# irvingzhang0512/tf_eager_object_detection

Measured on AMD Instinct MI355X. Metric: images/sec, higher is better.
Workload: dtype f32

## Files before the change

tf_eager_object_detection_amd/csrc/postops.hip:

```cpp
#include <mutex>

#include "odet_internal.h"

#define PO_THREADS 1024
#define PO_ROUND 128

typedef unsigned long long u64;

static int next_pow2_(int v) {
  int p = 1;
  while (p < v) p <<= 1;
  return p;
}

struct PostOpsParams {
  PerImg<const float*> scores_t;
  PerImg<const float*> deltas_t;
  PerImg<const float4*> rois_t;
  PerImg<const int32_t*> count_dev_t;
  int R, Ccls, P2, K;
  float means[4], stds[4];
  float wmax, hmax, min_edge, score_thr, nms_thr;
  float roi_div;
  PerImg<int32_t*> cls_count_t;
  PerImg<float4*> cls_boxes_t;
  PerImg<float*> cls_scores_t;
  PerImg<uint32_t*> ticket_t;
  int ncls1, max_per_image;
  int mode;
  PerImg<float4*> out_boxes_t;
  PerImg<int32_t*> out_labels_t;
  PerImg<float*> out_scores_t;
  PerImg<int32_t*> out_count_t;
  PerImg<float*> out_record_t;
};

__device__ __forceinline__ float key_to_score(uint32_t k) {
  const uint32_t asc = ~k;
  const uint32_t u = (asc & 0x80000000u) ? (asc & 0x7FFFFFFFu) : ~asc;
  return __uint_as_float(u);
}

struct MergeView {
  const int32_t* cls_count; const float4* cls_boxes; const float* cls_scores;
  int ncls1, K, max_per_image, mode;
  float4* out_boxes; int32_t* out_labels; float* out_scores; int32_t* out_count; float* out_record;
};

__device__ void postops_merge(const MergeView& p, unsigned char* smem) {
  uint32_t* key = reinterpret_cast<uint32_t*>(smem);
  const int nslots = p.ncls1 * p.K;
  uint32_t* hist = key + nslots;
  uint32_t* sel_key = hist + 256;
  uint32_t* sel_slot = sel_key + (p.max_per_image > 0 ? p.max_per_image : 1);
  __shared__ uint32_t s_prefix, s_target, s_total;
  __shared__ int lds17[17];
  const int tid = threadIdx.x, lane = tid & 63;
  const int per = (nslots + PO_THREADS - 1) / PO_THREADS;
  const int lo = tid * per;
  int nvalid = 0;
  for (int q = 0; q < per; ++q) {
    const int slot = lo + q;
    if (slot < nslots) {
      const int c = slot / p.K, k = slot - c * p.K;
      const float sc = p.cls_scores[slot];
      const bool valid = k < min(p.cls_count[c], p.K);
      key[slot] = valid ? ~d_float_asc_key(sc) : 0xFFFFFFFFu;
      nvalid += valid ? 1 : 0;
    }
  }
  int total;
  (void)block_excl_scan(nvalid, lds17, &total);
  const int M = (p.mode == 1) ? ((p.max_per_image > 0 && total > p.max_per_image) ? p.max_per_image : total)
                              : min(total, p.max_per_image);
  uint32_t T = 0xFFFFFFFFu;
  if (M > 0 && M < total) {
    if (tid == 0) { s_prefix = 0u; s_target = (uint32_t)M; }
    for (int pass = 0; pass < 4; ++pass) {
      const int shift = 24 - 8 * pass;
      if (tid < 256) hist[tid] = 0u;
      __syncthreads();
      const uint32_t prefix = s_prefix;
      const uint32_t himask = pass == 0 ? 0u : (0xFFFFFFFFu << (shift + 8));
      for (int q = 0; q < per; ++q) {
        const int slot = lo + q;
        if (slot < nslots) {
          const uint32_t k = key[slot];
          if (k != 0xFFFFFFFFu && (k & himask) == prefix) atomicAdd(&hist[(k >> shift) & 255u], 1u);
        }
      }
      __syncthreads();
      if (tid < 64) {
        const uint32_t h0 = hist[4 * tid], h1 = hist[4 * tid + 1], h2 = hist[4 * tid + 2], h3 = hist[4 * tid + 3];
        const int sum = (int)(h0 + h1 + h2 + h3);
        const int inc = wave_incl_scan(sum);
        const int tgt = (int)s_target;
        const bool hit = sum > 0 && inc - sum < tgt && tgt <= inc;
        const u64 bal = __ballot(hit);
        if (bal && lane == __builtin_ctzll(bal)) {
          int run = inc - sum;
          uint32_t d = 4 * tid;
          const uint32_t hh[4] = {h0, h1, h2, h3};
#pragma unroll
          for (int j = 0; j < 4; ++j) {
            if (run < tgt && tgt <= run + (int)hh[j]) { d = 4 * tid + j; s_target = (uint32_t)(tgt - run); }
            run += (int)hh[j];
          }
          s_prefix = prefix | (d << shift);
        }
      }
      __syncthreads();
    }
    T = s_prefix;
  }
  const uint32_t take_ties = (M > 0 && M < total) ? s_target : 0xFFFFFFFFu;
  __syncthreads();
  if (p.mode == 1) {
    int c = 0;
    for (int q = 0; q < per; ++q) {
      const int slot = lo + q;
      if (slot < nslots && key[slot] != 0xFFFFFFFFu && key[slot] <= T) ++c;
    }
    int kept_total;
    int o = block_excl_scan(c, lds17, &kept_total);
    for (int q = 0; q < per; ++q) {
      const int slot = lo + q;
      if (slot < nslots && key[slot] != 0xFFFFFFFFu && key[slot] <= T) {
        p.out_boxes[o] = p.cls_boxes[slot];
        p.out_scores[o] = p.cls_scores[slot];
        p.out_labels[o] = (int32_t)(slot / p.K) + 1;
        ++o;
      }
    }
    if (tid == 0) *p.out_count = kept_total;
    return;
  }
  int nlt = 0, neq = 0;
  for (int q = 0; q < per; ++q) {
    const int slot = lo + q;
    if (slot < nslots) {
      const uint32_t k = key[slot];
      if (k != 0xFFFFFFFFu) { nlt += (k < T || M == total) ? 1 : 0; neq += (k == T && M < total) ? 1 : 0; }
    }
  }
  int tot_eq, tot_lt;
  int eq_before = block_excl_scan(neq, lds17, &tot_eq);
  int sel_before = block_excl_scan(nlt + max(0, min(neq, (int)min((u64)take_ties, (u64)0x7FFFFFFF) - eq_before)), lds17, &tot_lt);
  {
    int o = sel_before, e = eq_before;
    for (int q = 0; q < per; ++q) {
      const int slot = lo + q;
      if (slot < nslots) {
        const uint32_t k = key[slot];
        bool sel = false;
        if (k != 0xFFFFFFFFu) {
          if (k < T || M == total) sel = true;
          else if (k == T) { sel = (uint32_t)e < take_ties; ++e; }
        }
        if (sel && o < M) { sel_key[o] = k; sel_slot[o] = (uint32_t)slot; ++o; }
      }
    }
  }
  __syncthreads();
  for (int i = tid; i < M; i += PO_THREADS) {
    const uint32_t ki = sel_key[i], si = sel_slot[i];
    int rank = 0;
    for (int j = 0; j < M; ++j) {
      const uint32_t kj = sel_key[j], sj = sel_slot[j];
      rank += (kj < ki || (kj == ki && sj < si)) ? 1 : 0;
    }
    const float4 b = p.cls_boxes[si];
    const float sc = p.cls_scores[si];
    const int lab = (int)(si / (uint32_t)p.K) + 1;
    p.out_boxes[rank] = b;
    p.out_scores[rank] = sc;
    p.out_labels[rank] = lab;
    if (p.out_record) {
      float* r = p.out_record + (size_t)rank * 6;
      r[0] = b.x; r[1] = b.y; r[2] = b.z; r[3] = b.w; r[4] = sc; r[5] = (float)lab;
    }
  }
  if (p.out_record) {
    for (int i = M + tid; i < p.max_per_image; i += PO_THREADS) {
      float* r = p.out_record + (size_t)i * 6;
      r[0] = 0.0f; r[1] = 0.0f; r[2] = 0.0f; r[3] = 0.0f; r[4] = -1.0f; r[5] = 0.0f;
    }
  }
  if (tid == 0) {
    *p.out_count = M;
    if (p.out_record) p.out_record[(size_t)p.max_per_image * 6] = (float)M;
  }
}

__global__ void __launch_bounds__(PO_THREADS) k_postops(PostOpsParams p) {
  extern __shared__ __align__(16) unsigned char smem[];
  const int img = blockIdx.y;
  const float* __restrict__ in_scores = p.scores_t.v[img];
  const float* __restrict__ in_deltas = p.deltas_t.v[img];
  const float4* __restrict__ in_rois = p.rois_t.v[img];
  const int32_t* __restrict__ in_count = p.count_dev_t.v[img];
  int32_t* __restrict__ cls_count = p.cls_count_t.v[img];
  float4* __restrict__ cls_boxes = p.cls_boxes_t.v[img];
  float* __restrict__ cls_scores = p.cls_scores_t.v[img];
  const int nkeys = p.P2 > 2048 ? p.P2 : 2048;
  u64* keys = reinterpret_cast<u64*>(smem);
  float4* lbox = reinterpret_cast<float4*>(keys + nkeys);
  float4* sbox = lbox + p.R;
  float4* kbox = sbox + PO_ROUND;
  u64* mask = reinterpret_cast<u64*>(kbox + p.K);
  float* sarea = reinterpret_cast<float*>(mask + PO_ROUND * 2);
  float* karea = sarea + PO_ROUND;
  uint32_t* crossf = reinterpret_cast<uint32_t*>(karea + p.K);
  __shared__ int s_nvalid, s_nk, s_last;

  const int c = blockIdx.x + 1;
  const int tid = threadIdx.x, lane = tid & 63, w = tid >> 6;
  if (tid == 0) { s_nvalid = 0; s_nk = 0; s_last = 0; }

  const int Rdev = in_count ? *in_count : p.R;
  u64 mykey = ~0ull;
  for (int r = tid; r < p.P2; r += PO_THREADS) {
    u64 key = ~0ull;
    if (r < p.R) {
      const float s = in_scores[(size_t)r * p.Ccls + c];
      const float4 t = *reinterpret_cast<const float4*>(in_deltas + ((size_t)r * p.Ccls + c) * 4);
      float4 roi = in_rois[r];
      if (r < min(Rdev, p.R) && s > p.score_thr) {
        const float d0 = t.x * p.stds[0] + p.means[0];
        const float d1 = t.y * p.stds[1] + p.means[1];
        const float d2 = t.z * p.stds[2] + p.means[2];
        const float d3 = t.w * p.stds[3] + p.means[3];
        if (p.roi_div != 1.0f) {
          roi.x = roi.x / p.roi_div; roi.y = roi.y / p.roi_div; roi.z = roi.z / p.roi_div; roi.w = roi.w / p.roi_div;
        }
        float4 b = d_decode_box(roi, d0, d1, d2, d3);
        b = d_clip_box(b, 0.0f, p.wmax, p.hmax);
        const float e0 = b.z - b.x + 1.0f, e1 = b.w - b.y + 1.0f;
        if (e1 >= p.min_edge && e0 >= p.min_edge) {
          lbox[r] = b;
          key = ((u64)(~d_float_asc_key(s)) << 32) | (unsigned)r;
        }
      }
    }
    if (p.P2 > 1024) keys[r] = key; else mykey = key;
  }
  __syncthreads();
  {
    const u64 bal = __ballot(p.P2 <= 1024 && mykey != ~0ull);
    if (lane == 0 && bal) atomicAdd(&s_nvalid, (int)__popcll(bal));
  }
  __syncthreads();

  if (p.P2 <= 1024) {
    mykey = bitonic_sort_1024_reg(mykey, keys);
    __syncthreads();
    keys[tid] = mykey;
    __syncthreads();
  } else {
    bitonic_sort_u64(keys, p.P2, PO_THREADS);
    if (tid == 0) {
      int lo = 0, hi = p.P2;
      while (lo < hi) { int mid = (lo + hi) >> 1; if (keys[mid] != ~0ull) lo = mid + 1; else hi = mid; }
      s_nvalid = lo;
    }
    __syncthreads();
  }
  const int nvalid = s_nvalid;
  const int K = p.K;

  const u64 lt_lane = (lane == 0) ? 0ull : (~0ull >> (64 - lane));
  for (int t0 = 0; t0 < nvalid; t0 += PO_ROUND) {
    const int nk0 = s_nk;
    if (nk0 >= K) break;
    const int mround = min(PO_ROUND, nvalid - t0);
    if (tid < PO_ROUND) {
      float4 nb = make_float4(0, 0, 0, 0);
      if (tid < mround) nb = d_norm_box(lbox[(int)(keys[t0 + tid] & 0xFFFFFFFFull)]);
      sbox[tid] = nb;
      sarea[tid] = d_box_area(nb);
      crossf[tid] = 0;
    }
    __syncthreads();
    {
      const int row = tid & (PO_ROUND - 1), cs = tid >> 7;
      const float4 rb = sbox[row];
      const float ra = sarea[row];
      uint32_t bits = 0;
#pragma unroll
      for (int j = 0; j < 16; ++j) {
        const int col = cs * 16 + j;
        const bool s = (col < row) && d_iou_gt(rb, ra, sbox[col], sarea[col], p.nms_thr);
        bits |= s ? (1u << j) : 0u;
      }
      reinterpret_cast<unsigned short*>(mask)[row * 8 + cs] = (unsigned short)bits;
      bool sup = false;
      for (int k = cs; k < nk0; k += 8) sup = sup || d_iou_gt(rb, ra, kbox[k], karea[k], p.nms_thr);
      if (sup) atomicOr(&crossf[row], 1u);
    }
    __syncthreads();
    if (w == 0) {
      int nk = nk0;
      u64 kept0 = 0;
#pragma unroll
      for (int blk = 0; blk < 2; ++blk) {
        const int row = blk * 64 + lane;
        const u64 m0 = mask[row * 2 + 0], m1 = mask[row * 2 + 1];
        bool dead = (row >= mround) || (crossf[row] != 0);
        if (blk == 1) dead = dead || ((m0 & kept0) != 0ull);
        const u64 mm = (blk == 0) ? m0 : m1;
        u64 alive = __ballot(!dead);
        u64 kept = 0;
        while (alive != 0 && nk < K) {
          const int i = __builtin_ctzll(alive);
          kept |= 1ull << i;
          ++nk;
          alive &= ~(1ull << i);
          alive &= ~__ballot((mm >> i) & 1ull);
        }
        if (blk == 0) kept0 = kept;
        if ((kept >> lane) & 1ull) {
          const int slot = nk0 + (blk == 1 ? (int)__popcll(kept0) : 0) + (int)__popcll(kept & lt_lane);
          const u64 kk = keys[t0 + row];
          const float4 ob = lbox[(int)(kk & 0xFFFFFFFFull)];
          kbox[slot] = sbox[row];
          karea[slot] = sarea[row];
          cls_boxes[(size_t)blockIdx.x * K + slot] = ob;
          cls_scores[(size_t)blockIdx.x * K + slot] = key_to_score((uint32_t)(kk >> 32));
        }
      }
      if (lane == 0) s_nk = nk;
    }
    __syncthreads();
  }
  if (tid == 0) cls_count[blockIdx.x] = s_nk;

  asm volatile("s_waitcnt vmcnt(0)" ::: "memory");
  __syncthreads();
  if (tid == 0) {
    __builtin_amdgcn_fence(__ATOMIC_RELEASE, "agent");
    asm volatile("s_waitcnt vmcnt(0)" ::: "memory");
    const uint32_t t = atomicInc(p.ticket_t.v[img], (uint32_t)(p.ncls1 - 1));
    s_last = (t == (uint32_t)(p.ncls1 - 1)) ? 1 : 0;
  }
  __syncthreads();
  if (!s_last) return;
  if (tid == 0) __builtin_amdgcn_fence(__ATOMIC_ACQUIRE, "agent");
  asm volatile("s_waitcnt vmcnt(0)" ::: "memory");
  __syncthreads();
  MergeView mv;
  mv.cls_count = cls_count; mv.cls_boxes = cls_boxes; mv.cls_scores = cls_scores;
  mv.ncls1 = p.ncls1; mv.K = p.K; mv.max_per_image = p.max_per_image; mv.mode = p.mode;
  mv.out_boxes = p.out_boxes_t.v[img]; mv.out_labels = p.out_labels_t.v[img]; mv.out_scores = p.out_scores_t.v[img];
  mv.out_count = p.out_count_t.v[img]; mv.out_record = p.out_record_t.v[img];
  postops_merge(mv, smem);
}

extern "C" size_t odet_post_ops_workspace_bytes(int num_classes, int max_per_class) {
  size_t n1 = (size_t)(num_classes > 1 ? num_classes - 1 : 1);
  size_t k = (size_t)(max_per_class > 0 ? max_per_class : 1);
  return odet_align_up(n1 * 4, 256) + odet_align_up(n1 * k * 16, 256) + odet_align_up(n1 * k * 4, 256) + 1024;
}

int odet_post_ops_batch(const PostOpsImageIO* io, int B, int R, int Ccls, int num_classes, PostOpsExtra ex,
                        const float* means, const float* stds, int max_per_class, int max_per_image,
                        float nms_iou_threshold, float score_threshold, float min_edge, hipStream_t st, int ws_clean) {
  ODET_REQUIRE(io && B >= 1 && B <= ODET_MAX_BATCH, "odet_post_ops: bad batch");
  ODET_REQUIRE(R >= 0 && Ccls > 0 && num_classes >= 1 && num_classes <= Ccls, "odet_post_ops: bad sizes");
  ODET_REQUIRE(max_per_class >= 0 && max_per_image >= 0, "odet_post_ops: negative cap");
  for (int i = 0; i < B; ++i) ODET_REQUIRE(io[i].out_count, "odet_post_ops: null out_count");
  if (R == 0 || num_classes == 1 || max_per_class == 0 || (max_per_image == 0 && ex.mode == 0)) {
    for (int i = 0; i < B; ++i) {
      ODET_HIP(hipMemsetAsync(io[i].out_count, 0, sizeof(int32_t), st));
      if (io[i].out_record && max_per_image > 0) {
        int rc = odet_pack_detections(io[i].out_boxes, io[i].out_labels, io[i].out_scores, io[i].out_count, 0,
                                      max_per_image, io[i].out_record, (odet_stream_t)st);
        if (rc != ODET_OK) return rc;
      }
    }
    return ODET_OK;
  }
  ODET_REQUIRE(means && stds, "odet_post_ops: null pointer");
  if (R > ODET_POSTOPS_MAX_ROIS)
    return odet_set_error(ODET_E_LIMIT, "odet_post_ops: R %d exceeds %d", R, ODET_POSTOPS_MAX_ROIS);
  const int ncls1 = num_classes - 1;
  if ((int64_t)ncls1 * max_per_class > ODET_POSTOPS_MAX_CANDIDATES)
    return odet_set_error(ODET_E_LIMIT, "odet_post_ops: (num_classes-1)*max_per_class %lld exceeds %d",
                          (long long)ncls1 * max_per_class, ODET_POSTOPS_MAX_CANDIDATES);
  const size_t need = odet_post_ops_workspace_bytes(num_classes, max_per_class);
  PostOpsParams p;
  for (int i = 0; i < ODET_MAX_BATCH; ++i) {
    const PostOpsImageIO& a = io[i < B ? i : 0];
    ODET_REQUIRE(a.scores && a.deltas && a.rois && a.out_boxes && a.out_labels && a.out_scores,
                 "odet_post_ops: null pointer");
    ODET_REQUIRE((uintptr_t)a.deltas % 16 == 0, "odet_post_ops: deltas must be 16-byte aligned");
    if (!a.workspace || a.workspace_bytes < need)
      return odet_set_error(ODET_E_WORKSPACE, "odet_post_ops: workspace too small (%zu < %zu)", a.workspace_bytes, need);
    OdetArena ar{(char*)a.workspace, a.workspace_bytes, 0};
    int32_t* cc = ar.take<int32_t>(ncls1);
    float4* cb = ar.take<float4>((size_t)ncls1 * max_per_class);
    float* cs = ar.take<float>((size_t)ncls1 * max_per_class);
    uint32_t* tk = ar.take<uint32_t>(1);
    ODET_REQUIRE(cc && cb && cs && tk, "odet_post_ops: workspace arena exhausted");
    p.scores_t.v[i] = a.scores; p.deltas_t.v[i] = a.deltas; p.rois_t.v[i] = (const float4*)a.rois;
    p.count_dev_t.v[i] = a.count_dev;
    p.cls_count_t.v[i] = cc; p.cls_boxes_t.v[i] = cb; p.cls_scores_t.v[i] = cs; p.ticket_t.v[i] = tk;
    p.out_boxes_t.v[i] = (float4*)a.out_boxes; p.out_labels_t.v[i] = a.out_labels; p.out_scores_t.v[i] = a.out_scores;
    p.out_count_t.v[i] = a.out_count; p.out_record_t.v[i] = a.out_record;
    if (!ws_clean && i < B) ODET_HIP(hipMemsetAsync(tk, 0, sizeof(uint32_t), st));
  }
  p.R = R; p.Ccls = Ccls; p.P2 = next_pow2_(R < 2 ? 2 : R); p.K = max_per_class;
  for (int k = 0; k < 4; ++k) { p.means[k] = means[k]; p.stds[k] = stds[k]; }
  p.wmax = ex.wmax; p.hmax = ex.hmax; p.roi_div = ex.roi_div;
  p.min_edge = min_edge; p.score_thr = score_threshold; p.nms_thr = nms_iou_threshold;
  p.ncls1 = ncls1; p.max_per_image = max_per_image; p.mode = ex.mode;
  const size_t nkeys1 = (size_t)(p.P2 > 2048 ? p.P2 : 2048);
  const size_t lds_class = nkeys1 * 8 + (size_t)R * 16 + PO_ROUND * 16 + (size_t)max_per_class * 16 + PO_ROUND * 16 +
                           PO_ROUND * 4 + (size_t)max_per_class * 4 + PO_ROUND * 4;
  const size_t lds_merge = (size_t)ncls1 * max_per_class * 4 + 256 * 4 + (size_t)(max_per_image > 0 ? max_per_image : 1) * 8 + 64;
  const size_t lds1 = lds_class > lds_merge ? lds_class : lds_merge;
  if (lds1 > 150 * 1024)
    return odet_set_error(ODET_E_LIMIT, "odet_post_ops: R/max_per_class need %zu B of LDS (> 150 KiB)", lds1);
  static OdetPerDeviceOnce once;
  ODET_HIP(once.run([] { return hipFuncSetAttribute((const void*)k_postops, hipFuncAttributeMaxDynamicSharedMemorySize, 150 * 1024); }));
  hipLaunchKernelGGL(k_postops, dim3(ncls1, B), dim3(PO_THREADS), lds1, st, p);
  ODET_LAUNCH_CHECK();
  return ODET_OK;
}

static int post_ops_impl(const float* scores, const float* deltas, const float* rois, int R,
                         const int32_t* count_dev, int Ccls, int num_classes, PostOpsExtra ex,
                         const float* means, const float* stds, int max_per_class, int max_per_image,
                         float nms_iou_threshold, float score_threshold, float min_edge, float* out_boxes,
                         int32_t* out_labels, float* out_scores, int32_t* out_count, float* out_record,
                         void* workspace, size_t workspace_bytes, hipStream_t st) {
  PostOpsImageIO io{scores, deltas, rois, count_dev, out_boxes, out_labels, out_scores, out_count, out_record,
                    workspace, workspace_bytes};
  ODET_REQUIRE(out_count, "odet_post_ops: null out_count");
  return odet_post_ops_batch(&io, 1, R, Ccls, num_classes, ex, means, stds, max_per_class, max_per_image,
                             nms_iou_threshold, score_threshold, min_edge, st,  0);
}

extern "C" int odet_post_ops(const float* scores, const float* deltas, const float* rois, int R,
                             const int32_t* count_dev, int Ccls, int num_classes, int image_h, int image_w,
                             const float* means, const float* stds, int max_per_class, int max_per_image,
                             float nms_iou_threshold, float score_threshold, float min_edge, float* out_boxes,
                             int32_t* out_labels, float* out_scores, int32_t* out_count, void* workspace,
                             size_t workspace_bytes, odet_stream_t stream) {
  ODET_REQUIRE(image_h > 0 && image_w > 0, "odet_post_ops: bad image shape");
  return post_ops_impl(scores, deltas, rois, R, count_dev, Ccls, num_classes,
                       PostOpsExtra{(float)(image_w - 1), (float)(image_h - 1), 1.0f, 0}, means, stds,
                       max_per_class, max_per_image, nms_iou_threshold, score_threshold, min_edge, out_boxes,
                       out_labels, out_scores, out_count, nullptr, workspace, workspace_bytes, (hipStream_t)stream);
}

extern "C" int odet_eval_detect(const float* scores, const float* deltas, const float* rois, int R,
                                const int32_t* count_dev, int Ccls, int num_classes, float img_scale, float raw_h,
                                float raw_w, const float* means, const float* stds, int max_per_class,
                                int max_per_image, float nms_iou_threshold, float score_threshold, float min_size,
                                float* out_boxes, int32_t* out_labels, float* out_scores, int32_t* out_count,
                                void* workspace, size_t workspace_bytes, odet_stream_t stream) {
  ODET_REQUIRE(img_scale > 0.0f && raw_h > 0.0f && raw_w > 0.0f, "odet_eval_detect: bad scale / image size");
  return post_ops_impl(scores, deltas, rois, R, count_dev, Ccls, num_classes,
                       PostOpsExtra{raw_w - 1.0f, raw_h - 1.0f, img_scale, 1}, means, stds, max_per_class,
                       max_per_image, nms_iou_threshold, score_threshold, min_size, out_boxes, out_labels,
                       out_scores, out_count, nullptr, workspace, workspace_bytes, (hipStream_t)stream);
}

extern "C" int odet_eval_detect_topk(const float* scores, const float* deltas, const float* rois, int R,
                                     const int32_t* count_dev, int Ccls, int num_classes, float img_scale, float raw_h,
                                     float raw_w, const float* means, const float* stds, int max_per_class,
                                     int max_per_image, float nms_iou_threshold, float score_threshold, float min_size,
                                     float* out_boxes, int32_t* out_labels, float* out_scores, int32_t* out_count,
                                     void* workspace, size_t workspace_bytes, odet_stream_t stream) {
  ODET_REQUIRE(img_scale > 0.0f && raw_h > 0.0f && raw_w > 0.0f, "odet_eval_detect_topk: bad scale / image size");
  return post_ops_impl(scores, deltas, rois, R, count_dev, Ccls, num_classes,
                       PostOpsExtra{raw_w - 1.0f, raw_h - 1.0f, img_scale, 0}, means, stds, max_per_class,
                       max_per_image, nms_iou_threshold, score_threshold, min_size, out_boxes, out_labels,
                       out_scores, out_count, nullptr, workspace, workspace_bytes, (hipStream_t)stream);
}

extern "C" int odet_post_ops_record(const float* scores, const float* deltas, const float* rois, int R,
                                    const int32_t* count_dev, int Ccls, int num_classes, int image_h, int image_w,
                                    const float* means, const float* stds, int max_per_class, int max_per_image,
                                    float nms_iou_threshold, float score_threshold, float min_edge,
                                    float* out_boxes, int32_t* out_labels, float* out_scores, int32_t* out_count,
                                    float* out_record, void* workspace, size_t workspace_bytes,
                                    odet_stream_t stream) {
  ODET_REQUIRE(out_record, "odet_post_ops_record: null out_record");
  ODET_REQUIRE(image_h > 0 && image_w > 0, "odet_post_ops_record: bad image shape");
  return post_ops_impl(scores, deltas, rois, R, count_dev, Ccls, num_classes,
                       PostOpsExtra{(float)(image_w - 1), (float)(image_h - 1), 1.0f, 0}, means, stds,
                       max_per_class, max_per_image, nms_iou_threshold, score_threshold, min_edge, out_boxes,
                       out_labels, out_scores, out_count, out_record, workspace, workspace_bytes,
                       (hipStream_t)stream);
}

__global__ void __launch_bounds__(256) k_pack_detections(const float4* __restrict__ boxes,
                                                         const int32_t* __restrict__ labels,
                                                         const float* __restrict__ scores,
                                                         const int32_t* __restrict__ count, int cap, int max_det,
                                                         float* __restrict__ rec) {
  const int m = min(min(*count, cap), max_det);
  for (int i = threadIdx.x; i < max_det; i += 256) {
    float* r = rec + (size_t)i * 6;
    if (i < m) {
      float4 b = boxes[i];
      r[0] = b.x; r[1] = b.y; r[2] = b.z; r[3] = b.w; r[4] = scores[i]; r[5] = (float)labels[i];
    } else {
      r[0] = 0.0f; r[1] = 0.0f; r[2] = 0.0f; r[3] = 0.0f; r[4] = -1.0f; r[5] = 0.0f;
    }
  }
  if (threadIdx.x == 0) rec[(size_t)max_det * 6] = (float)m;
}

extern "C" int odet_pack_detections(const float* boxes, const int32_t* labels, const float* scores,
                                    const int32_t* count_dev, int capacity, int max_det, float* out_record,
                                    odet_stream_t stream) {
  ODET_REQUIRE(boxes && labels && scores && count_dev && out_record, "odet_pack_detections: null pointer");
  ODET_REQUIRE(capacity >= 0 && max_det > 0, "odet_pack_detections: bad sizes");
  hipLaunchKernelGGL(k_pack_detections, dim3(1), dim3(256), 0, (hipStream_t)stream, (const float4*)boxes, labels,
                     scores, count_dev, capacity, max_det, out_record);
  ODET_LAUNCH_CHECK();
  return ODET_OK;
}
```

Baseline: 29620.

## Replace full bitonic sort with per-round radix select and lazy box decode

The per-class NMS kernel no longer sorts all R candidate keys with a bitonic sort and decodes every box up front. Each round it picks the next top PO_ROUND candidates with a four-pass radix select, ranks them within the round, and decodes only those boxes. Block size and round size drop to 512 threads and 64 rows, which shrinks LDS use and may allow more blocks per CU. The cost is a radix select pass over all R keys every round, which can add up when many rounds run before K boxes are kept.

```diff
diff --git a/tf_eager_object_detection_amd/csrc/postops.hip b/tf_eager_object_detection_amd/csrc/postops.hip
--- a/tf_eager_object_detection_amd/csrc/postops.hip
+++ b/tf_eager_object_detection_amd/csrc/postops.hip
@@ -2,23 +2,27 @@
 
 #include "odet_internal.h"
 
-#define PO_THREADS 1024
-#define PO_ROUND 128
+#ifndef PO_THREADS
+#define PO_THREADS 512
+#endif
+#ifndef PO_ROUND
+#define PO_ROUND 64
+#endif
+#define PO_SLICES (PO_THREADS / PO_ROUND)
+#define PO_COLS (PO_ROUND / PO_SLICES)
+#define PO_WORDS (PO_ROUND / 64)
+#define PO_INVALID 0xFFFFFFFFu
+static_assert((PO_THREADS == 256 || PO_THREADS == 512) && (PO_ROUND == 64 || PO_ROUND == 128), "k_postops: unsupported shape");
+static_assert(PO_COLS == 8 || PO_COLS == 16 || PO_COLS == 32 || PO_COLS == 64, "k_postops: mask pieces are 1, 2, 4 or 8 bytes");
 
 typedef unsigned long long u64;
-
-static int next_pow2_(int v) {
-  int p = 1;
-  while (p < v) p <<= 1;
-  return p;
-}
 
 struct PostOpsParams {
   PerImg<const float*> scores_t;
   PerImg<const float*> deltas_t;
   PerImg<const float4*> rois_t;
   PerImg<const int32_t*> count_dev_t;
-  int R, Ccls, P2, K;
+  int R, Ccls, K;
   float means[4], stds[4];
   float wmax, hmax, min_edge, score_thr, nms_thr;
   float roi_div;
@@ -41,6 +45,42 @@
   return __uint_as_float(u);
 }
 
+__device__ __forceinline__ uint32_t po_radix_select(const uint32_t* key, int n, int M, uint32_t* hist, uint32_t* ties) {
+  const int tid = threadIdx.x, lane = tid & 63;
+  for (int i = tid; i < 4 * 256; i += PO_THREADS) hist[i] = 0u;
+  __syncthreads();
+  uint32_t prefix = 0u;
+  int tgt = M;
+  for (int pass = 0; pass < 4; ++pass) {
+    const int shift = 24 - 8 * pass;
+    uint32_t* h = hist + pass * 256;
+    const uint32_t himask = pass == 0 ? 0u : (0xFFFFFFFFu << (shift + 8));
+    for (int i = tid; i < n; i += PO_THREADS) {
+      const uint32_t k = key[i];
+      if (k != PO_INVALID && (k & himask) == prefix) atomicAdd(&h[(k >> shift) & 255u], 1u);
+    }
+    __syncthreads();
+    const uint4 hv = reinterpret_cast<const uint4*>(h)[lane];
+    const uint32_t hh[4] = {hv.x, hv.y, hv.z, hv.w};
+    const int sum = (int)(hv.x + hv.y + hv.z + hv.w);
+    const int inc = wave_incl_scan(sum);
+    const bool hit = sum > 0 && inc - sum < tgt && tgt <= inc;
+    int run = inc - sum, nt = tgt;
+    uint32_t d = 4 * lane;
+#pragma unroll
+    for (int j = 0; j < 4; ++j) {
+      if (run < tgt && tgt <= run + (int)hh[j]) { d = 4 * lane + j; nt = tgt - run; }
+      run += (int)hh[j];
+    }
+    const u64 bal = __ballot(hit);
+    const int src = bal ? __builtin_ctzll(bal) : 0;
+    prefix |= (uint32_t)__shfl((int)d, src) << shift;
+    tgt = __shfl(nt, src);
+  }
+  *ties = (uint32_t)tgt;
+  return prefix;
+}
+
 struct MergeView {
   const int32_t* cls_count; const float4* cls_boxes; const float* cls_scores;
   int ncls1, K, max_per_image, mode;
@@ -50,12 +90,11 @@
 __device__ void postops_merge(const MergeView& p, unsigned char* smem) {
   uint32_t* key = reinterpret_cast<uint32_t*>(smem);
   const int nslots = p.ncls1 * p.K;
-  uint32_t* hist = key + nslots;
-  uint32_t* sel_key = hist + 256;
-  uint32_t* sel_slot = sel_key + (p.max_per_image > 0 ? p.max_per_image : 1);
-  __shared__ uint32_t s_prefix, s_target, s_total;
+  uint32_t* hist = key + ((nslots + 3) & ~3);
+  uint32_t* sel_key = hist + 4 * 256;
+  uint32_t* sel_slot = sel_key + max(min(p.max_per_image, nslots), 1);
   __shared__ int lds17[17];
-  const int tid = threadIdx.x, lane = tid & 63;
+  const int tid = threadIdx.x;
   const int per = (nslots + PO_THREADS - 1) / PO_THREADS;
   const int lo = tid * per;
   int nvalid = 0;
@@ -73,47 +112,8 @@
   (void)block_excl_scan(nvalid, lds17, &total);
   const int M = (p.mode == 1) ? ((p.max_per_image > 0 && total > p.max_per_image) ? p.max_per_image : total)
                               : min(total, p.max_per_image);
-  uint32_t T = 0xFFFFFFFFu;
-  if (M > 0 && M < total) {
-    if (tid == 0) { s_prefix = 0u; s_target = (uint32_t)M; }
-    for (int pass = 0; pass < 4; ++pass) {
-      const int shift = 24 - 8 * pass;
-      if (tid < 256) hist[tid] = 0u;
-      __syncthreads();
-      const uint32_t prefix = s_prefix;
-      const uint32_t himask = pass == 0 ? 0u : (0xFFFFFFFFu << (shift + 8));
-      for (int q = 0; q < per; ++q) {
-        const int slot = lo + q;
-        if (slot < nslots) {
-          const uint32_t k = key[slot];
-          if (k != 0xFFFFFFFFu && (k & himask) == prefix) atomicAdd(&hist[(k >> shift) & 255u], 1u);
-        }
-      }
-      __syncthreads();
-      if (tid < 64) {
-        const uint32_t h0 = hist[4 * tid], h1 = hist[4 * tid + 1], h2 = hist[4 * tid + 2], h3 = hist[4 * tid + 3];
-        const int sum = (int)(h0 + h1 + h2 + h3);
-        const int inc = wave_incl_scan(sum);
-        const int tgt = (int)s_target;
-        const bool hit = sum > 0 && inc - sum < tgt && tgt <= inc;
-        const u64 bal = __ballot(hit);
-        if (bal && lane == __builtin_ctzll(bal)) {
-          int run = inc - sum;
-          uint32_t d = 4 * tid;
-          const uint32_t hh[4] = {h0, h1, h2, h3};
-#pragma unroll
-          for (int j = 0; j < 4; ++j) {
-            if (run < tgt && tgt <= run + (int)hh[j]) { d = 4 * tid + j; s_target = (uint32_t)(tgt - run); }
-            run += (int)hh[j];
-          }
-          s_prefix = prefix | (d << shift);
-        }
-      }
-      __syncthreads();
-    }
-    T = s_prefix;
-  }
-  const uint32_t take_ties = (M > 0 && M < total) ? s_target : 0xFFFFFFFFu;
+  uint32_t T = PO_INVALID, take_ties = PO_INVALID;
+  if (M > 0 && M < total) T = po_radix_select(key, nslots, M, hist, &take_ties);
   __syncthreads();
   if (p.mode == 1) {
     int c = 0;
@@ -202,30 +202,97 @@
   int32_t* __restrict__ cls_count = p.cls_count_t.v[img];
   float4* __restrict__ cls_boxes = p.cls_boxes_t.v[img];
   float* __restrict__ cls_scores = p.cls_scores_t.v[img];
-  const int nkeys = p.P2 > 2048 ? p.P2 : 2048;
-  u64* keys = reinterpret_cast<u64*>(smem);
-  float4* lbox = reinterpret_cast<float4*>(keys + nkeys);
-  float4* sbox = lbox + p.R;
-  float4* kbox = sbox + PO_ROUND;
+  float4* sbox = reinterpret_cast<float4*>(smem);
+  float4* obox = sbox + PO_ROUND;
+  float4* kbox = obox + PO_ROUND;
   u64* mask = reinterpret_cast<u64*>(kbox + p.K);
-  float* sarea = reinterpret_cast<float*>(mask + PO_ROUND * 2);
+  uint32_t* hist = reinterpret_cast<uint32_t*>(mask + PO_ROUND * PO_WORDS);
+  uint32_t* key = hist + 4 * 256;
+  uint32_t* bkey = key + p.R;
+  uint32_t* brow = bkey + PO_ROUND;
+  uint32_t* skey = brow + PO_ROUND;
+  uint32_t* crossf = skey + PO_ROUND;
+  float* sarea = reinterpret_cast<float*>(crossf + PO_ROUND);
   float* karea = sarea + PO_ROUND;
-  uint32_t* crossf = reinterpret_cast<uint32_t*>(karea + p.K);
   __shared__ int s_nvalid, s_nk, s_last;
+  __shared__ int lds17[17];
 
   const int c = blockIdx.x + 1;
   const int tid = threadIdx.x, lane = tid & 63, w = tid >> 6;
   if (tid == 0) { s_nvalid = 0; s_nk = 0; s_last = 0; }
+  __syncthreads();
 
   const int Rdev = in_count ? *in_count : p.R;
-  u64 mykey = ~0ull;
-  for (int r = tid; r < p.P2; r += PO_THREADS) {
-    u64 key = ~0ull;
-    if (r < p.R) {
-      const float s = in_scores[(size_t)r * p.Ccls + c];
-      const float4 t = *reinterpret_cast<const float4*>(in_deltas + ((size_t)r * p.Ccls + c) * 4);
-      float4 roi = in_rois[r];
-      if (r < min(Rdev, p.R) && s > p.score_thr) {
+  {
+    int nv = 0;
+    for (int r0 = tid; r0 < p.R; r0 += 4 * PO_THREADS) {
+      float s[4];
+#pragma unroll
+      for (int u = 0; u < 4; ++u) {
+        const int r = r0 + u * PO_THREADS;
+        s[u] = r < p.R ? in_scores[(size_t)r * p.Ccls + c] : 0.0f;
+      }
+#pragma unroll
+      for (int u = 0; u < 4; ++u) {
+        const int r = r0 + u * PO_THREADS;
+        const bool ok = r < min(Rdev, p.R) && s[u] > p.score_thr;
+        if (r < p.R) key[r] = ok ? ~d_float_asc_key(s[u]) : PO_INVALID;
+        nv += ok ? 1 : 0;
+      }
+    }
+    nv = wave_incl_scan(nv);
+    if (lane == 63 && nv) atomicAdd(&s_nvalid, nv);
+  }
+  __syncthreads();
+  const int nvalid = s_nvalid;
+  const int K = p.K;
+  const int per = (p.R + PO_THREADS - 1) / PO_THREADS;
+  const int lo = tid * per;
+  const u64 lt_lane = (lane == 0) ? 0ull : (~0ull >> (64 - lane));
+
+  for (int taken = 0; taken < nvalid; taken += PO_ROUND) {
+    const int nk0 = s_nk;
+    if (nk0 >= K) break;
+    const int left = nvalid - taken;
+    const int mround = min(PO_ROUND, left);
+    uint32_t T = PO_INVALID, ties = 0u;
+    if (mround < left) T = po_radix_select(key, p.R, mround, hist, &ties);
+    int nlt = 0, neq = 0;
+    for (int q = 0; q < per; ++q) {
+      const int row = lo + q;
+      if (row < p.R) {
+        const uint32_t k = key[row];
+        nlt += (k < T) ? 1 : 0;
+        neq += (k == T && k != PO_INVALID) ? 1 : 0;
+      }
+    }
+    {
+      int tot;
+      const int before = block_excl_scan(nlt | (neq << 16), lds17, &tot);
+      int e = before >> 16;
+      int o = (before & 0xFFFF) + min(e, (int)ties);
+      for (int q = 0; q < per; ++q) {
+        const int row = lo + q;
+        if (row < p.R) {
+          const uint32_t k = key[row];
+          bool sel = k < T;
+          if (k == T && k != PO_INVALID) { sel = e < (int)ties; ++e; }
+          if (sel && o < PO_ROUND) { bkey[o] = k; brow[o] = (uint32_t)row; key[row] = PO_INVALID; ++o; }
+        }
+      }
+    }
+    __syncthreads();
+    if (tid < PO_ROUND) {
+      if (tid < mround) {
+        const uint32_t ki = bkey[tid];
+        const int r = (int)brow[tid];
+        const float4 t = *reinterpret_cast<const float4*>(in_deltas + ((size_t)r * p.Ccls + c) * 4);
+        float4 roi = in_rois[r];
+        int rank = 0;
+        for (int j = 0; j < mround; ++j) {
+          const uint32_t kj = bkey[j];
+          rank += (kj < ki || (kj == ki && j < tid)) ? 1 : 0;
+        }
         const float d0 = t.x * p.stds[0] + p.means[0];
         const float d1 = t.y * p.stds[1] + p.means[1];
         const float d2 = t.z * p.stds[2] + p.means[2];
@@ -236,65 +303,37 @@
         float4 b = d_decode_box(roi, d0, d1, d2, d3);
         b = d_clip_box(b, 0.0f, p.wmax, p.hmax);
         const float e0 = b.z - b.x + 1.0f, e1 = b.w - b.y + 1.0f;
-        if (e1 >= p.min_edge && e0 >= p.min_edge) {
-          lbox[r] = b;
-          key = ((u64)(~d_float_asc_key(s)) << 32) | (unsigned)r;
-        }
-      }
-    }
-    if (p.P2 > 1024) keys[r] = key; else mykey = key;
-  }
-  __syncthreads();
-  {
-    const u64 bal = __ballot(p.P2 <= 1024 && mykey != ~0ull);
-    if (lane == 0 && bal) atomicAdd(&s_nvalid, (int)__popcll(bal));
-  }
-  __syncthreads();
-
-  if (p.P2 <= 1024) {
-    mykey = bitonic_sort_1024_reg(mykey, keys);
-    __syncthreads();
-    keys[tid] = mykey;
-    __syncthreads();
-  } else {
-    bitonic_sort_u64(keys, p.P2, PO_THREADS);
-    if (tid == 0) {
-      int lo = 0, hi = p.P2;
-      while (lo < hi) { int mid = (lo + hi) >> 1; if (keys[mid] != ~0ull) lo = mid + 1; else hi = mid; }
-      s_nvalid = lo;
-    }
-    __syncthreads();
-  }
-  const int nvalid = s_nvalid;
-  const int K = p.K;
-
-  const u64 lt_lane = (lane == 0) ? 0ull : (~0ull >> (64 - lane));
-  for (int t0 = 0; t0 < nvalid; t0 += PO_ROUND) {
-    const int nk0 = s_nk;
-    if (nk0 >= K) break;
-    const int mround = min(PO_ROUND, nvalid - t0);
-    if (tid < PO_ROUND) {
-      float4 nb = make_float4(0, 0, 0, 0);
-      if (tid < mround) nb = d_norm_box(lbox[(int)(keys[t0 + tid] & 0xFFFFFFFFull)]);
-      sbox[tid] = nb;
-      sarea[tid] = d_box_area(nb);
-      crossf[tid] = 0;
+        const bool ok = e1 >= p.min_edge && e0 >= p.min_edge;
+        const float4 nb = d_norm_box(b);
+        sbox[rank] = nb;
+        obox[rank] = b;
+        sarea[rank] = d_box_area(nb);
+        skey[rank] = ki;
+        crossf[rank] = ok ? 0u : 1u;
+      } else {
+        sbox[tid] = make_float4(0, 0, 0, 0);
+        sarea[tid] = 0.0f;
+        crossf[tid] = 1u;
+      }
     }
     __syncthreads();
     {
-      const int row = tid & (PO_ROUND - 1), cs = tid >> 7;
+      const int row = tid & (PO_ROUND - 1), cs = tid / PO_ROUND;
       const float4 rb = sbox[row];
       const float ra = sarea[row];
-      uint32_t bits = 0;
+      u64 bits = 0;
 #pragma unroll
-      for (int j = 0; j < 16; ++j) {
-        const int col = cs * 16 + j;
+      for (int j = 0; j < PO_COLS; ++j) {
+        const int col = cs * PO_COLS + j;
         const bool s = (col < row) && d_iou_gt(rb, ra, sbox[col], sarea[col], p.nms_thr);
-        bits |= s ? (1u << j) : 0u;
-      }
-      reinterpret_cast<unsigned short*>(mask)[row * 8 + cs] = (unsigned short)bits;
+        bits |= s ? (1ull << j) : 0ull;
+      }
+      if (PO_COLS == 8) reinterpret_cast<unsigned char*>(mask)[row * PO_SLICES + cs] = (unsigned char)bits;
+      else if (PO_COLS == 16) reinterpret_cast<unsigned short*>(mask)[row * PO_SLICES + cs] = (unsigned short)bits;
+      else if (PO_COLS == 32) reinterpret_cast<uint32_t*>(mask)[row * PO_SLICES + cs] = (uint32_t)bits;
+      else mask[row * PO_SLICES + cs] = bits;
       bool sup = false;
-      for (int k = cs; k < nk0; k += 8) sup = sup || d_iou_gt(rb, ra, kbox[k], karea[k], p.nms_thr);
+      for (int k = cs; k < nk0; k += PO_SLICES) sup = sup || d_iou_gt(rb, ra, kbox[k], karea[k], p.nms_thr);
       if (sup) atomicOr(&crossf[row], 1u);
     }
     __syncthreads();
@@ -302,9 +341,9 @@
       int nk = nk0;
       u64 kept0 = 0;
 #pragma unroll
-      for (int blk = 0; blk < 2; ++blk) {
+      for (int blk = 0; blk < PO_WORDS; ++blk) {
         const int row = blk * 64 + lane;
-        const u64 m0 = mask[row * 2 + 0], m1 = mask[row * 2 + 1];
+        const u64 m0 = mask[row * PO_WORDS + 0], m1 = mask[row * PO_WORDS + PO_WORDS - 1];
         bool dead = (row >= mround) || (crossf[row] != 0);
         if (blk == 1) dead = dead || ((m0 & kept0) != 0ull);
         const u64 mm = (blk == 0) ? m0 : m1;
@@ -320,12 +359,10 @@
         if (blk == 0) kept0 = kept;
         if ((kept >> lane) & 1ull) {
           const int slot = nk0 + (blk == 1 ? (int)__popcll(kept0) : 0) + (int)__popcll(kept & lt_lane);
-          const u64 kk = keys[t0 + row];
-          const float4 ob = lbox[(int)(kk & 0xFFFFFFFFull)];
           kbox[slot] = sbox[row];
           karea[slot] = sarea[row];
-          cls_boxes[(size_t)blockIdx.x * K + slot] = ob;
-          cls_scores[(size_t)blockIdx.x * K + slot] = key_to_score((uint32_t)(kk >> 32));
+          cls_boxes[(size_t)blockIdx.x * K + slot] = obox[row];
+          cls_scores[(size_t)blockIdx.x * K + slot] = key_to_score(skey[row]);
         }
       }
       if (lane == 0) s_nk = nk;
@@ -408,15 +445,16 @@
     p.out_count_t.v[i] = a.out_count; p.out_record_t.v[i] = a.out_record;
     if (!ws_clean && i < B) ODET_HIP(hipMemsetAsync(tk, 0, sizeof(uint32_t), st));
   }
-  p.R = R; p.Ccls = Ccls; p.P2 = next_pow2_(R < 2 ? 2 : R); p.K = max_per_class;
+  p.R = R; p.Ccls = Ccls; p.K = max_per_class;
   for (int k = 0; k < 4; ++k) { p.means[k] = means[k]; p.stds[k] = stds[k]; }
   p.wmax = ex.wmax; p.hmax = ex.hmax; p.roi_div = ex.roi_div;
   p.min_edge = min_edge; p.score_thr = score_threshold; p.nms_thr = nms_iou_threshold;
   p.ncls1 = ncls1; p.max_per_image = max_per_image; p.mode = ex.mode;
-  const size_t nkeys1 = (size_t)(p.P2 > 2048 ? p.P2 : 2048);
-  const size_t lds_class = nkeys1 * 8 + (size_t)R * 16 + PO_ROUND * 16 + (size_t)max_per_class * 16 + PO_ROUND * 16 +
-                           PO_ROUND * 4 + (size_t)max_per_class * 4 + PO_ROUND * 4;
-  const size_t lds_merge = (size_t)ncls1 * max_per_class * 4 + 256 * 4 + (size_t)(max_per_image > 0 ? max_per_image : 1) * 8 + 64;
+  const size_t lds_class = 2 * PO_ROUND * 16 + (size_t)max_per_class * 16 + PO_ROUND * PO_WORDS * 8 + 4 * 256 * 4 +
+                           (size_t)R * 4 + 5 * PO_ROUND * 4 + (size_t)max_per_class * 4;
+  const size_t nslots = (size_t)ncls1 * max_per_class;
+  const size_t nsel = max_per_image > 0 ? ((size_t)max_per_image < nslots ? (size_t)max_per_image : nslots) : 1;
+  const size_t lds_merge = nslots * 4 + 4 * 256 * 4 + nsel * 8 + 64;
   const size_t lds1 = lds_class > lds_merge ? lds_class : lds_merge;
   if (lds1 > 150 * 1024)
     return odet_set_error(ODET_E_LIMIT, "odet_post_ops: R/max_per_class need %zu B of LDS (> 150 KiB)", lds1);
```

Result: faster. 30150 (median of 6 runs) (+1.8%).
